# Sin3DM/Sin3DM

Hardware: AMD Instinct MI355X
Metric: DDPM-1000 triplane samples/sec @128^2 latent (higher is better)
Workload: dtype f32; 1 GPU; BASELINE configs[1]: 128^2 triplane (H,W,D)=(128,128,128), 128-ch TriplaneUNetModelSmall, DDPM-1000, batch 1 per GPU; a step = 1 denoising step; batch_per_gpu=1, parallelism=1 independent samples, prewarm_steps=150

## Files before the change

### include/sin3dm_hip.h

```cpp
#ifndef SIN3DM_HIP_H
#define SIN3DM_HIP_H

#include <stddef.h>
#include <stdint.h>

#ifdef __cplusplus
extern "C" {
#endif

#define S3D_ABI_VERSION 13
#define S3D_API __attribute__((visibility("default")))

typedef enum {
    S3D_OK = 0,
    S3D_ERR_INVALID = -1,
    S3D_ERR_MISSING = -2,
    S3D_ERR_HIP = -3,
    S3D_ERR_UNSUPPORTED = -4,
    S3D_ERR_INTERNAL = -5
} s3d_status;

S3D_API int s3d_abi_version(void);

S3D_API int s3d_set_option(const char* name, const char* value);
S3D_API int s3d_get_option(const char* name, int* value);
S3D_API int s3d_set_riders(int on);
S3D_API const char* s3d_last_error(void);
S3D_API int s3d_device_count(void);

typedef struct s3d_unet s3d_unet;

typedef struct {
    int32_t in_channels;
    int32_t model_channels;
    int32_t out_channels;
    int32_t num_res_blocks;
    int32_t n_levels;
    int32_t channel_mult[8];
    int32_t use_scale_shift_norm;
    int32_t is_rollout;
} s3d_unet_cfg;
// ... 18 lines not shown
S3D_API int s3d_unet_forward_film(s3d_unet* m, const float* x, const float* film, int film_stride, int B, int H, int W, int D,
                          float* out, void* stream);

#define S3D_PROF_CLASSES 4
typedef struct {
    double ms[S3D_PROF_CLASSES];
    double flops[S3D_PROF_CLASSES];
    int64_t launches[S3D_PROF_CLASSES];
    int64_t forwards;
    double mfma_flops[S3D_PROF_CLASSES];
} s3d_profile;
S3D_API int s3d_unet_profile(s3d_unet* m, int every);
S3D_API int s3d_unet_profile_classes(s3d_unet* m, int mask);
S3D_API int s3d_unet_profile_read(s3d_unet* m, s3d_profile* out);
S3D_API const char* s3d_unet_profile_kernel(const s3d_unet* m, int cls);
enum { S3D_TAB_SQRT_RECIP = 0, S3D_TAB_SQRT_RECIPM1, S3D_TAB_COEF1, S3D_TAB_COEF2, S3D_TAB_LOGVAR,
       S3D_TAB_ACP, S3D_TAB_ACP_PREV, S3D_TAB_ROWS };
enum { S3D_STEP_DDPM = 0, S3D_STEP_DDIM = 1, S3D_STEP_MEAN_ONLY = 2 };
enum { S3D_MEAN_START_X = 0, S3D_MEAN_EPSILON = 1 };

typedef struct {
    int32_t mode;
    int32_t mean_type;
    int32_t clip_denoised;
    int32_t is_mask_t0;
    float eta;
    int32_t T;
    int64_t batch;
    int64_t per_sample;
    const float* model_out;
// ... 237 lines not shown
```

### sin3dm_amd/_lib.py

```python
from __future__ import annotations

import ctypes as C
import os

_HERE = os.path.dirname(os.path.abspath(__file__))
LIB_PATH = os.path.join(_HERE, "libsin3dm_hip.so")

c_fp = C.POINTER(C.c_float)
c_i64p = C.POINTER(C.c_int64)

ABI_VERSION = 13
TAB_ROWS = ("sqrt_recip", "sqrt_recipm1", "coef1", "coef2", "logvar", "acp", "acp_prev")
KTAB_ROWS = ("sqrt_acp_prev", "sqrt_1m_acp_prev", "sqrt_1m_beta", "sqrt_beta")
STEP_DDPM, STEP_DDIM, STEP_MEAN_ONLY = 0, 1, 2
CARRY_OUT, CARRY_IN = 1, 2
MEAN_START_X, MEAN_EPSILON = 0, 1
ERR_INVALID, ERR_MISSING, ERR_HIP, ERR_UNSUPPORTED, ERR_INTERNAL = -1, -2, -3, -4, -5
MAX_LANES = 16
MESHSDF_MAX_PAIRS = 1 << 27
RENDER_MAX_PAIRS = 1 << 27
RENDER_TILE, RENDER_SUBPIXEL, RENDER_MAX_COORD, RENDER_MAX_GRID = 16, 256, 1 << 20, 4096
IMGFEAT_INCEPTION, IMGFEAT_ALEXNET = 0, 1
RENDER_AMBIENT, RENDER_DIFFUSE = 0.35, 0.65

# ... 29 lines not shown
                ("tex_threshold_ratio", C.c_float), ("tex_weight", C.c_float)]


class DecoderCfg(C.Structure):
    _fields_ = [("geo_feat_channels", C.c_int32), ("tex_feat_channels", C.c_int32), ("feat_channel_up", C.c_int32),
                ("mlp_hidden_channels", C.c_int32), ("mlp_hidden_layers", C.c_int32), ("tex_channels", C.c_int32)]


SIGNATURES = {
    "s3d_abi_version": (C.c_int, []),
    "s3d_last_error": (C.c_char_p, []),
    "s3d_device_count": (C.c_int, []),
    "s3d_set_option": (C.c_int, [C.c_char_p, C.c_char_p]),
    "s3d_get_option": (C.c_int, [C.c_char_p, C.POINTER(C.c_int)]),
    "s3d_set_riders": (C.c_int, [C.c_int]),
    "s3d_unet_create": (C.c_int, [C.POINTER(UNetCfg), C.POINTER(C.c_void_p)]),
    "s3d_unet_destroy": (None, [C.c_void_p]),
    "s3d_unet_num_params": (C.c_int, [C.c_void_p]),
    "s3d_unet_param_info": (C.c_int, [C.c_void_p, C.c_int, C.POINTER(C.c_char_p), c_i64p, C.POINTER(C.c_int)]),
    "s3d_unet_set_param": (C.c_int, [C.c_void_p, C.c_char_p, C.c_void_p, c_i64p, C.c_int]),
    "s3d_unet_forward": (C.c_int, [C.c_void_p, C.c_void_p, C.c_void_p, C.c_int, C.c_int, C.c_int, C.c_int,
                                   C.c_void_p, C.c_void_p]),
    "s3d_unet_film_width": (C.c_int, [C.c_void_p]),
    "s3d_unet_film": (C.c_int, [C.c_void_p, C.c_void_p, C.c_int, C.c_void_p, C.c_void_p]),
    "s3d_unet_select_lane": (C.c_int, [C.c_void_p, C.c_int]),
    "s3d_unet_current_lane": (C.c_int, [C.c_void_p]),
    "s3d_unet_forward_film": (C.c_int, [C.c_void_p, C.c_void_p, C.c_void_p, C.c_int, C.c_int, C.c_int, C.c_int, C.c_int,
                                        C.c_void_p, C.c_void_p]),
    "s3d_unet_profile": (C.c_int, [C.c_void_p, C.c_int]),
    "s3d_unet_profile_classes": (C.c_int, [C.c_void_p, C.c_int]),
    "s3d_unet_profile_read": (C.c_int, [C.c_void_p, C.POINTER(Profile)]),
    "s3d_unet_profile_kernel": (C.c_char_p, [C.c_void_p, C.c_int]),
    "s3d_sampler_step": (C.c_int, [C.POINTER(SamplerArgs), C.c_void_p]),
    "s3d_unet_step_film": (C.c_int, [C.c_void_p, C.c_void_p, C.c_int, C.c_int, C.c_int, C.c_int, C.c_int,
                                     C.POINTER(SamplerArgs), C.c_void_p, C.c_void_p]),
    "s3d_unet_step_film_carry": (C.c_int, [C.c_void_p, C.c_void_p, C.c_int, C.c_int, C.c_int, C.c_int, C.c_int,
                                           C.POINTER(SamplerArgs), C.c_void_p, C.c_void_p, C.c_int]),
    "s3d_sampler_step_known": (C.c_int, [C.POINTER(SamplerArgs), C.POINTER(KnownRegionArgs), C.c_void_p]),
    "s3d_unet_step_film_known": (C.c_int, [C.c_void_p, C.c_void_p, C.c_int, C.c_int, C.c_int, C.c_int, C.c_int,
                                           C.POINTER(SamplerArgs), C.POINTER(KnownRegionArgs), C.c_void_p, C.c_void_p, C.c_int]),
    "s3d_sampler_renoise": (C.c_int, [C.c_void_p, C.c_void_p, C.c_void_p, C.c_void_p, C.c_int32, C.c_int64, C.c_int64, C.c_void_p,
                                      C.c_void_p]),
    "s3d_op_triplane_conv": (C.c_int, [C.POINTER(C.c_void_p), C.POINTER(C.c_void_p), C.c_int, C.c_int, C.c_int,
                                       C.c_int, C.c_int, C.c_int, C.c_int, C.c_int, C.POINTER(C.c_void_p),
                                       C.POINTER(C.c_void_p), C.c_void_p]),
    "s3d_op_triplane_norm_silu": (C.c_int, [C.POINTER(C.c_void_p), C.POINTER(C.c_void_p), C.c_int, C.c_int, C.c_int,
                                            C.c_int, C.c_int, C.POINTER(C.c_void_p), C.POINTER(C.c_void_p),
# ... 180 lines not shown
    if not torch.cuda.is_available():
        raise Sin3DMHipError("sin3dm_amd needs a visible MI355X (torch.cuda.is_available() is False); "
                             "there is no CPU fallback")


def set_option(name, value):
    check(load().s3d_set_option(str(name).encode(), None if value is None else str(value).encode()))


def get_option(name):
    v = C.c_int(0)
    check(load().s3d_get_option(str(name).encode(), C.byref(v)))
    return None if v.value == -1 else v.value


def set_riders(on):
    check(load().s3d_set_riders(1 if on else 0))


def stream_ptr():
    import torch
    return C.c_void_p(torch.cuda.current_stream().cuda_stream)


def ptr(t):
    return C.c_void_p(t.data_ptr()) if t is not None else C.c_void_p(0)


def ptr3(ts):
    return (C.c_void_p * 3)(*[C.c_void_p(t.data_ptr()) for t in ts])
# ... 1 lines not shown
```

### sin3dm_amd/csrc/s3d_common.h

```cpp
#pragma once
#include <hip/hip_runtime.h>

#include <atomic>
#include <cstdarg>
#include <cstdint>
#include <cstdio>
#include <cstring>
#include <map>
#include <string>
#include <vector>

#include "../../include/sin3dm_hip.h"

namespace s3d {

void set_error(const char* fmt, ...) __attribute__((format(printf, 1, 2)));
const char* get_error();

#define S3D_HIP(call)                                                                              \
    do {                                                                                           \
        hipError_t e__ = (call);                                                                   \
        if (e__ != hipSuccess) {                                                                   \
            s3d::set_error("%s failed: %s (%s:%d)", #call, hipGetErrorString(e__), __FILE__, __LINE__); \
            return S3D_ERR_HIP;                                                                    \
// ... 138 lines not shown
    const float* u[3];
    int hi[3], wi[3];
    int C, cq, pl, sg, nsub, maxparts;
    double* part;
};
struct GnFinCatArgs {
    const double* pu; const double* ps; float* mr;
    int maxparts_u, maxparts_s, nparts_u[3], nparts_s[3], nsub_u, nsub_s, subs_per_group;
    double count[3];
};
enum RiderKind { RIDER_NONE = 0, RIDER_GN_PARTIALS_UP, RIDER_GN_FINALIZE, RIDER_GN_FINALIZE_CAT };
struct ConvRider {
    int kind;
    int n_blocks;
    int gx;
    union { GnPartUpArgs up; GnFinArgs fin; GnFinCatArgs cat; };
};
constexpr int kRiderLdsBytes = 16384;
int launch_conv(ConvKind kind, ConvArgs& a, hipStream_t st, const ConvRider* rider = nullptr);
bool conv1x1_takes_rider(const Geo& g, int B, int cout);
int launch_conv_naive(ConvKind kind, ConvArgs& a, hipStream_t st);
bool conv_use_naive();
void conv_note_kernel(const char* name);
const char* conv_last_kernel();
double conv_exec_fraction(ConvKind kind, const ConvArgs& a);

struct ConvW {
    size_t dense[3] = {0, 0, 0};
    size_t bias[3] = {0, 0, 0};
    size_t rrow[3] = {0, 0, 0};
// ... 48 lines not shown
bool conv_use_wino24();
bool conv_wino24_channels(int cin, int cout);
size_t wino24_packed_floats(int cout, int cin);
size_t pack_wino24s_weights(std::vector<float>& stage, const float* W, int cout, int ctot, int cin);
int launch_conv_wino24s(ConvArgs& a, hipStream_t st);
int launch_conv_wino24_narrow(ConvArgs& a, hipStream_t st);
int launch_conv_wino24_wide(ConvArgs& a, hipStream_t st);

struct ActArgs {
    const float* gamma[3];
    const float* beta[3];
    const float* film;
    int film_stride;
};
constexpr int kActRows = 8, kActCols = 8;
struct MeanPartials {
    float* rowpart[3];
    float* colpart[3];
};
int launch_gn_act(const Tri& x, int B, GnStats stats, const ActArgs& a, Tri& y, const MeanPartials* mp,
                  hipStream_t st, const GnPartials* stats_part = nullptr);
bool gn_act_can_add_parts(const GnPartials& part, int C);
bool gn_parts_in_consumer(long long consumer_blocks);
int gn_act_threads(int C);
long long gn_act_blocks(const Geo& g, int B);
int launch_gn_finalize_as(const GnPartials& part, const Geo& g, int C, int B, int threads, GnStats out, hipStream_t st);
int launch_gn_act_cat(const Tri& u, const Tri& sk, int B, GnStats stats, const ActArgs& a, Tri& y, const MeanPartials* mp,
                      hipStream_t st);
struct MeanVecs { float* rowmean[3]; float* colmean[3]; };
struct MeanFinArgs {
// ... 40 lines not shown
```

### sin3dm_amd/csrc/s3d_conv.hip

```cpp
#include "s3d_common.h"
#include "s3d_rank1.h"
#include "s3d_riders.h"

namespace s3d {

typedef float f32x16 __attribute__((ext_vector_type(16)));

#ifndef S3D_ABLATE
#define S3D_ABLATE 0
#endif
constexpr int KC = 32;
constexpr int LDP = KC + 4;

__device__ __forceinline__ float up2x_blend(float ly0, float ly1, float lx0, float lx1, float v00, float v01, float v10, float v11) {
    const float top = __fmaf_rn(lx1, v01, __fmul_rn(lx0, v00));
    const float bot = __fmaf_rn(lx1, v11, __fmul_rn(lx0, v10));
    return __fmaf_rn(ly1, bot, __fmul_rn(ly0, top));
}

template <int TH_, int TW_, int KH_, int KW_, int WM_, int WN_, int MTW_, int NTW_, int KS_ = 1, int PF_ = 0, bool TR_ = false>
struct ConvCfg {
    static constexpr int KS = KS_;
    static constexpr int PF = PF_;
    static constexpr bool TR = TR_;
// ... 18 lines not shown

template <bool RIDER> struct RiderArg {};
template <> struct RiderArg<true> { ConvRider r; };
template <class CFG, bool RIDER = false>
__global__ __launch_bounds__(256) void k_conv_mfma(ConvArgs args, RiderArg<RIDER> rider) {
    constexpr int TW = CFG::TW, KH = CFG::KH, KW = CFG::KW, MTW = CFG::MTW, NTW = CFG::NTW;
    constexpr int HW = CFG::HW, TAPS = KH * KW;
    __shared__ __attribute__((aligned(16))) float smem[2 * (CFG::A_ELEMS + CFG::B_ELEMS)];
    float* const Abase = smem;
    float* const Bbase = smem + 2 * CFG::A_ELEMS;

    int bid = blockIdx.x;
    int nblocks = gridDim.x;
    if constexpr (RIDER) {
        static_assert(sizeof smem >= size_t(kRiderLdsBytes) && KH == 1 && !CFG::TR, "the rider bodies work in the 1x1 convolution's LDS");
        if (bid < rider.r.n_blocks) { run_rider(rider.r, bid, smem); return; }
        bid -= rider.r.n_blocks; nblocks -= rider.r.n_blocks;
    }
    if (args.xcd_swizzle) {
        const int chunk = nblocks >> 3;
        if (bid < (chunk << 3)) bid = (bid & 7) * chunk + (bid >> 3);
    }
    int j = 0;
#pragma unroll
    for (int k = 1; k < kMaxConvJobs; ++k) j += (k < args.njobs && bid >= args.job[k].block_begin) ? 1 : 0;
    const ConvJob& J = args.job[j];
    int local = bid - J.block_begin;
    const int ntile = local % J.n_tiles_n; local /= J.n_tiles_n;
    const int b = local / J.tiles_per_img; local %= J.tiles_per_img;
    const int ty0 = (local / J.tiles_x) * CFG::TH, tx0 = (local % J.tiles_x) * TW;
    const int n0 = ntile * CFG::BN;
    const int h = J.h, w = J.w, cin = args.cin, cout = args.cout;
// ... 724 lines not shown
```

### sin3dm_amd/csrc/s3d_kernels.hip

```cpp
#include "s3d_common.h"
#include "s3d_rank1.h"
#include "s3d_riders.h"
#include "s3d_sampler.h"

namespace s3d {

__device__ __forceinline__ float silu_f(float v) { return v * __builtin_amdgcn_rcpf(1.0f + __expf(-v)); }

static inline int cdiv(int a, int b) { return (a + b - 1) / b; }

__global__ void k_nchw_to_nhwc(const float* __restrict__ in, float* __restrict__ out, int B, int C, int hw) {
    size_t i = size_t(blockIdx.x) * blockDim.x + threadIdx.x;
    size_t n = size_t(B) * C * hw;
    if (i >= n) return;
    int c = int(i % C);
    size_t r = i / C;
    int pix = int(r % hw);
    int b = int(r / hw);
    out[i] = in[(size_t(b) * C + c) * hw + pix];
}
__global__ void k_nhwc_to_nchw(const float* __restrict__ in, float* __restrict__ out, int B, int C, int hw) {
    size_t i = size_t(blockIdx.x) * blockDim.x + threadIdx.x;
    size_t n = size_t(B) * C * hw;
    if (i >= n) return;
// ... 213 lines not shown

__global__ __launch_bounds__(256) void k_gn_finalize(GnFinArgs a) {
    __shared__ double sm4[4];
    gn_finalize_block(a, blockIdx.x, blockIdx.y, blockIdx.z, sm4);
}
static bool gn_finalize_args(const GnPartials& part, const Geo& g, int C, GnStats out, GnFinArgs& a) {
    a.part = part.p; a.mr = out.mr; a.maxparts = part.maxparts; a.nsub = part.nsub;
    if (part.nsub % 32 != 0) return false;
    a.subs_per_group = part.nsub / 32;
    for (int p = 0; p < 3; ++p) { a.nparts[p] = part.nparts[p]; a.count[p] = double(C / 32) * g.h[p] * g.w[p]; }
    return true;
}
bool gn_finalize_rider(const GnPartials& part, const Geo& g, int C, int B, GnStats out, ConvRider& r) {
    memset(&r, 0, sizeof r);
    if (!B || !gn_finalize_args(part, g, C, out, r.fin)) return false;
    r.kind = RIDER_GN_FINALIZE; r.gx = 32; r.n_blocks = 32 * 3 * B;
    return true;
}
int launch_gn_finalize(const GnPartials& part, const Geo& g, int C, int B, GnStats out, hipStream_t st) {
    GnFinArgs a;
    S3D_CHECK(gn_finalize_args(part, g, C, out, a), S3D_ERR_INVALID, "gn_finalize: nsub=%d", part.nsub);
    if (!B) return 0;
    hipLaunchKernelGGL(k_gn_finalize, dim3(32, 3, B), dim3(256), 0, st, a);
    S3D_HIP(hipGetLastError());
    return 0;
}

__device__ __forceinline__ float4 up2x_sample(const float4* __restrict__ src, int hi, int wi, int cuq, int yo, int xo) {
    float fy = 0.5f * (float(yo) + 0.5f) - 0.5f; fy = fy < 0.f ? 0.f : fy;
    float fx = 0.5f * (float(xo) + 0.5f) - 0.5f; fx = fx < 0.f ? 0.f : fx;
    int y0 = int(fy); y0 = y0 > hi - 1 ? hi - 1 : y0;
// ... 30 lines not shown
int launch_gn_partials_up(const Tri& u, int B, int sg, GnPartials out, hipStream_t st) {
    GnPartUpArgs a;
    int maxtiles = 0;
    S3D_CHECK(gn_partials_up_args(u, sg, out, a, maxtiles), S3D_ERR_INVALID, "gn_partials_up: layout");
    if (!maxtiles || !B) return 0;
    hipLaunchKernelGGL(k_gn_partials_up, dim3(maxtiles, 3, B), dim3(a.cq * a.pl), size_t(a.pl) * a.C * 2 * sizeof(double), st, a);
    S3D_HIP(hipGetLastError());
    return 0;
}
bool gn_partials_up_rider(const Tri& u, int B, int sg, GnPartials out, ConvRider& r) {
    memset(&r, 0, sizeof r);
    int maxtiles = 0;
    if (!gn_partials_up_args(u, sg, out, r.up, maxtiles) || !maxtiles || !B) return false;
    if (r.up.cq * r.up.pl != 256 || size_t(r.up.pl) * r.up.C * 2 * sizeof(double) > size_t(kRiderLdsBytes)) return false;
    r.kind = RIDER_GN_PARTIALS_UP; r.gx = maxtiles; r.n_blocks = maxtiles * 3 * B;
    return true;
}
__global__ __launch_bounds__(256) void k_gn_finalize_cat(GnFinCatArgs a) {
    __shared__ double sm4[4];
    gn_finalize_cat_block(a, blockIdx.x, blockIdx.y, blockIdx.z, sm4);
}
static bool gn_finalize_cat_args(const GnPartials& pu, const GnPartials& ps, const Geo& g, int C, GnStats out, GnFinCatArgs& a) {
    a.pu = pu.p; a.ps = ps.p; a.mr = out.mr; a.maxparts_u = pu.maxparts; a.maxparts_s = ps.maxparts; a.nsub_u = pu.nsub; a.nsub_s = ps.nsub;
    if ((pu.nsub + ps.nsub) % 32 != 0) return false;
    a.subs_per_group = (pu.nsub + ps.nsub) / 32;
    for (int p = 0; p < 3; ++p) { a.nparts_u[p] = pu.nparts[p]; a.nparts_s[p] = ps.nparts[p]; a.count[p] = double(C / 32) * g.h[p] * g.w[p]; }
    return true;
}
bool gn_finalize_cat_rider(const GnPartials& pu, const GnPartials& ps, const Geo& g, int C, int B, GnStats out, ConvRider& r) {
    memset(&r, 0, sizeof r);
    if (!B || !gn_finalize_cat_args(pu, ps, g, C, out, r.cat)) return false;
    r.kind = RIDER_GN_FINALIZE_CAT; r.gx = 32; r.n_blocks = 32 * 3 * B;
    return true;
}
int launch_gn_finalize_cat(const GnPartials& pu, const GnPartials& ps, const Geo& g, int C, int B, GnStats out, hipStream_t st) {
    GnFinCatArgs a;
    S3D_CHECK(gn_finalize_cat_args(pu, ps, g, C, out, a), S3D_ERR_INVALID, "gn_finalize_cat: nsub=%d+%d", pu.nsub, ps.nsub);
    if (!B) return 0;
    hipLaunchKernelGGL(k_gn_finalize_cat, dim3(32, 3, B), dim3(256), 0, st, a);
    S3D_HIP(hipGetLastError());
    return 0;
}

struct GnPartSrc { const double* part; int nparts[3], maxparts, nsub, spg; double count[3]; };
__device__ __forceinline__ float* gn_stats_from_parts(const GnPartSrc& a, int b, int p, double* sd, float* mr_out) {
    const int L = int(blockDim.x) >> 5, tid = threadIdx.x;
    if (tid < 32 * L) {
// ... 51 lines not shown
    hipLaunchKernelGGL(k_gn_finalize_as, dim3(3, B), dim3(threads), size_t(threads) * 2 * sizeof(double) + 64 * sizeof(float), st, ps, out.mr);
    S3D_HIP(hipGetLastError());
    return 0;
}

struct GnActArgs {
    const float* x[3]; float* y[3];
    const float* gamma[3]; const float* beta[3];
    float* rowpart[3]; float* colpart[3];
    const float* mr;
    const float* film; int film_stride;
    int h[3], w[3];
    int C, cq, pl, with_means;
    GnPartSrc ps;
    float* mr_out;
};
__global__ __launch_bounds__(256) void k_gn_act(GnActArgs a) {
    extern __shared__ __attribute__((aligned(16))) char smem_raw[];
    float* sm = reinterpret_cast<float*>(smem_raw);
    const int p = blockIdx.y, b = blockIdx.z;
    const int h = a.h[p], w = a.w[p];
    const int ntc = (w + kActCols - 1) / kActCols, ntr = (h + kActRows - 1) / kActRows;
    if (int(blockIdx.x) >= ntc * ntr) return;
    const int tr = blockIdx.x / ntc, tc = blockIdx.x % ntc;
    const bool ident = a.mr == nullptr && a.ps.part == nullptr;
    const int q = threadIdx.x % a.cq, l = threadIdx.x / a.cq;
    const int i0 = tr * kActRows, j0 = tc * kActCols;
    const int i1 = min(h, i0 + kActRows), j1 = min(w, j0 + kActCols);
    const float4* xs = reinterpret_cast<const float4*>(a.x[p] + size_t(b) * h * w * a.C) + q;
    float4* ys = reinterpret_cast<float4*>(a.y[p] + size_t(b) * h * w * a.C) + q;
    float4 xfirst[kActRows];
    {
        const int j = min(j0 + l, j1 - 1);
#pragma unroll
        for (int r = 0; r < kActRows; ++r) xfirst[r] = xs[(size_t(min(i0 + r, i1 - 1)) * w + j) * a.cq];
    }
    const bool film = a.film != nullptr;
    float4 gam4 = make_float4(1, 1, 1, 1), bet4 = make_float4(0, 0, 0, 0), fsc4 = make_float4(0, 0, 0, 0), fsh4 = make_float4(0, 0, 0, 0);
    if (!ident) { gam4 = reinterpret_cast<const float4*>(a.gamma[p])[q]; bet4 = reinterpret_cast<const float4*>(a.beta[p])[q]; }
    if (film) {
        fsc4 = reinterpret_cast<const float4*>(a.film + size_t(b) * a.film_stride)[q];
// ... 15 lines not shown
        const float s1[4] = {fsc4.x, fsc4.y, fsc4.z, fsc4.w}, s2[4] = {fsh4.x, fsh4.y, fsh4.z, fsh4.w};
#pragma unroll
        for (int k = 0; k < 4; ++k) {
            const int c = 4 * q + k, g = c / cg;
            const float scale = ident ? 1.0f : sm[32 + g] * gv[k];
            A[k] = scale;
            Bc[k] = ident ? 0.0f : bv[k] - scale * sm[g];
            sc[k] = film ? 1.0f + s1[k] : 1.0f;
            sh[k] = film ? s2[k] : 0.0f;
        }
    }
    __syncthreads();
    float4 rowacc[kActRows];
#pragma unroll
    for (int r = 0; r < kActRows; ++r) rowacc[r] = make_float4(0, 0, 0, 0);
    for (int j = j0 + l; j < j1; j += a.pl) {
        float4 colacc = make_float4(0, 0, 0, 0);
        float4 xin[kActRows];
        if (j == j0 + l) {
#pragma unroll
            for (int r = 0; r < kActRows; ++r) xin[r] = xfirst[r];
        } else {
#pragma unroll
            for (int r = 0; r < kActRows; ++r) xin[r] = xs[(size_t(min(i0 + r, i1 - 1)) * w + j) * a.cq];
        }
#pragma unroll
        for (int r = 0; r < kActRows; ++r) {
            const int i = i0 + r;
            if (i < i1) {
                const size_t off = (size_t(i) * w + j) * a.cq;
                const float4 v = xin[r];
                float4 o;
                o.x = fmaf(v.x, A[0], Bc[0]); o.y = fmaf(v.y, A[1], Bc[1]);
                o.z = fmaf(v.z, A[2], Bc[2]); o.w = fmaf(v.w, A[3], Bc[3]);
// ... 1 lines not shown
                    o.x = o.x * sc[0] + sh[0]; o.y = o.y * sc[1] + sh[1];
                    o.z = o.z * sc[2] + sh[2]; o.w = o.w * sc[3] + sh[3];
                }
                if (!ident) { o.x = silu_f(o.x); o.y = silu_f(o.y); o.z = silu_f(o.z); o.w = silu_f(o.w); }
                ys[off] = o;
                colacc.x += o.x; colacc.y += o.y; colacc.z += o.z; colacc.w += o.w;
                rowacc[r].x += o.x; rowacc[r].y += o.y; rowacc[r].z += o.z; rowacc[r].w += o.w;
            }
        }
        if (a.with_means)
            reinterpret_cast<float4*>(a.colpart[p] + ((size_t(b) * ntr + tr) * w + j) * a.C)[q] = colacc;
    }
    if (!a.with_means) return;
    float4* smr = reinterpret_cast<float4*>(smem_raw);
#pragma unroll
    for (int r = 0; r < kActRows; ++r) smr[(size_t(l) * kActRows + r) * a.cq + q] = rowacc[r];
    __syncthreads();
    const int nthr = a.cq * a.pl;
    for (int it = threadIdx.x; it < kActRows * a.cq; it += nthr) {
        const int r = it / a.cq, qq = it % a.cq;
        const int i = i0 + r;
        if (i >= i1) continue;
        float4 s = make_float4(0, 0, 0, 0);
        for (int ll = 0; ll < a.pl; ++ll) {
            const float4 v = smr[(size_t(ll) * kActRows + r) * a.cq + qq];
            s.x += v.x; s.y += v.y; s.z += v.z; s.w += v.w;
        }
        reinterpret_cast<float4*>(a.rowpart[p] + ((size_t(b) * ntc + tc) * h + i) * a.C)[qq] = s;
    }
}
bool gn_act_can_add_parts(const GnPartials& part, int C) {
    if (!part.p || part.nsub % 32 != 0 || C % 32 != 0) return false;
    return (part.nsub / 32) * part.maxparts <= 160;
}
bool gn_parts_in_consumer(long long consumer_blocks) {
    const int mode = opt(OPT_GN_FUSED);
    const int cus = device_cus();
    return mode < 0 ? consumer_blocks <= 6LL * cus : mode != 0;
}
int gn_act_threads(int C) { int cq, pl; thread_shape(C, cq, pl); return cq * std::min(pl, kActCols); }
long long gn_act_blocks(const Geo& g, int B) {
    int maxtiles = 0;
    for (int p = 0; p < 3; ++p) maxtiles = std::max(maxtiles, cdiv(g.h[p], kActRows) * cdiv(g.w[p], kActCols));
// ... 9 lines not shown
        a.ps = gn_part_src(*stats_part, x.g, x.C);
    }
    int maxtiles = 0;
    for (int p = 0; p < 3; ++p) {
        a.x[p] = x.p[p]; a.y[p] = y.p[p]; a.h[p] = x.g.h[p]; a.w[p] = x.g.w[p];
        a.gamma[p] = aa.gamma[p]; a.beta[p] = aa.beta[p];
        a.rowpart[p] = mp ? mp->rowpart[p] : nullptr;
        a.colpart[p] = mp ? mp->colpart[p] : nullptr;
        maxtiles = std::max(maxtiles, cdiv(a.h[p], kActRows) * cdiv(a.w[p], kActCols));
    }
    a.mr = stats.mr; a.film = aa.film; a.film_stride = aa.film_stride;
    a.C = x.C; thread_shape(x.C, a.cq, a.pl); a.with_means = mp ? 1 : 0;
    a.pl = std::min(a.pl, kActCols);
    S3D_CHECK(x.C % 32 == 0 && a.cq * a.pl <= 256, S3D_ERR_INVALID, "GroupNorm(32, C): C=%d unsupported", x.C);
    if (!maxtiles || !B) return 0;
    size_t shm = std::max(size_t(64) * sizeof(float), size_t(a.pl) * kActRows * a.C * sizeof(float));
    if (a.ps.part) shm = std::max(shm, size_t(a.cq) * a.pl * 2 * sizeof(double) + 64 * sizeof(float));
    hipLaunchKernelGGL(k_gn_act, dim3(maxtiles, 3, B), dim3(a.cq * a.pl), shm, st, a);
    S3D_HIP(hipGetLastError());
    return 0;
}

struct GnActCatArgs {
    GnActArgs base;
    const float* u[3]; const float* sk[3];
    int cuq, csq;
};
__global__ __launch_bounds__(512) void k_gn_act_cat(GnActCatArgs ca) {
    const GnActArgs& a = ca.base;
    extern __shared__ __attribute__((aligned(16))) char smem_raw[];
    float* sm = reinterpret_cast<float*>(smem_raw);
    const int p = blockIdx.y, b = blockIdx.z;
    const int h = a.h[p], w = a.w[p];
// ... 98 lines not shown
    int maxtiles = 0;
    for (int p = 0; p < 3; ++p) {
        a.x[p] = nullptr; a.y[p] = y.p[p]; a.h[p] = y.g.h[p]; a.w[p] = y.g.w[p];
        ca.u[p] = u.p[p]; ca.sk[p] = sk.p[p];
        a.gamma[p] = aa.gamma[p]; a.beta[p] = aa.beta[p];
        a.rowpart[p] = mp ? mp->rowpart[p] : nullptr;
        a.colpart[p] = mp ? mp->colpart[p] : nullptr;
        maxtiles = std::max(maxtiles, cdiv(a.h[p], kActRows) * cdiv(a.w[p], kActCols));
        S3D_CHECK(y.g.h[p] == 2 * u.g.h[p] && y.g.w[p] == 2 * u.g.w[p] && sk.g.h[p] == y.g.h[p] && sk.g.w[p] == y.g.w[p], S3D_ERR_INVALID, "gn_act_cat: geometry");
    }
    ca.cuq = u.C / 4; ca.csq = sk.C / 4;
    a.mr = stats.mr; a.film = aa.film; a.film_stride = aa.film_stride;
    a.C = y.C; thread_shape(y.C, a.cq, a.pl); a.with_means = mp ? 1 : 0;
    S3D_CHECK(y.C == u.C + sk.C && y.C % 32 == 0 && a.cq * a.pl <= 512 && stats.mr, S3D_ERR_INVALID, "gn_act_cat: C=%d unsupported", y.C);
    if (!maxtiles || !B) return 0;
    size_t shm = std::max(size_t(64) * sizeof(float), size_t(a.pl) * kActRows * a.C * sizeof(float));
    hipLaunchKernelGGL(k_gn_act_cat, dim3(maxtiles, 3, B), dim3(a.cq * a.pl), shm, st, ca);
    S3D_HIP(hipGetLastError());
    return 0;
}

__global__ __launch_bounds__(256) void k_means_finalize(MeanFinArgs a) {
    means_finalize_thread(a, blockIdx.y, blockIdx.z, int(blockIdx.x * 128 + threadIdx.x));
}
MeanFinArgs means_finalize_args(const Geo& g, int C, int B, const MeanPartials& mp, const MeanVecs& mv) {
    MeanFinArgs a;
    a.C = C; a.cq = C / 4; a.B = B;
    for (int p = 0; p < 3; ++p) {
        const int h = g.h[p], w = g.w[p];
        a.src[2 * p] = mp.rowpart[p]; a.dst[2 * p] = mv.rowmean[p];
// ... 746 lines not shown
```

### sin3dm_amd/csrc/s3d_model.h

```cpp
#pragma once
#include <algorithm>
#include <cmath>
#include <memory>

#include "s3d_common.h"

namespace s3d {

static const char* kPlane[3] = {"xy", "xz", "yz"};

struct ParamSpec {
    std::string name;
    std::vector<int64_t> shape;
    size_t numel() const { size_t n = 1; for (auto d : shape) n *= size_t(d); return n; }
};

struct NormW { size_t gamma[3], beta[3]; };
struct ResBlockW {
    std::string prefix;
    int C, Cout;
    NormW n1, n2;
    ConvW c1, c2, skip;
    ConvW skip_a, skip_b;
    int c_up = 0;
// ... 100 lines not shown
    struct ProfRec { int cls; hipEvent_t e0, e1; double flops, mfma_flops; };
    int prof_every = 0;
    long fwd_count = 0;
    bool prof_now = false;
    int prof_mask = 15;
    bool prof_train = false;
    std::vector<ProfRec> prof_recs;
    std::vector<hipEvent_t> prof_pool;
    int64_t prof_forwards = 0;
    std::string prof_kernel[S3D_PROF_CLASSES];
    void note_prof_kernel(int cls) {
        if (cls < 0 || cls >= S3D_PROF_CLASSES) return;
        const std::string n = conv_last_kernel();
        if (n.empty() || prof_kernel[cls].find(n) != std::string::npos) return;
        prof_kernel[cls] += (prof_kernel[cls].empty() ? "" : " + ") + n;
    }
    hipEvent_t prof_event() {
        hipEvent_t e = nullptr;
        if (!prof_pool.empty()) { e = prof_pool.back(); prof_pool.pop_back(); }
        else if (hipEventCreate(&e) != hipSuccess) e = nullptr;
        return e;
    }
    int timed_conv(int cls, ConvKind kind, ConvArgs& ca, hipStream_t st, const ConvRider* rider = nullptr) {
        if (!prof_now || !((prof_mask >> cls) & 1)) return launch_conv(kind, ca, st, rider);
        int taps = kind == CONV_3x3 ? 9 : (kind == CONV_1x1 ? 1 : (kind == CONV_1x3_VEC ? 3 : (kind == CONV_1x3_ROLL ? 9 : 25)));
        double pix = 0;
        for (int j = 0; j < ca.njobs; ++j) pix += double(ca.job[j].h) * ca.job[j].w;
        ProfRec r{cls, prof_event(), prof_event(), 2.0 * taps * ca.cin * ca.cout * pix * ca.B, 0.0};
        r.mfma_flops = r.flops * conv_exec_fraction(kind, ca);
        if (r.e0) (void)hipEventRecord(r.e0, st);
// ... 133 lines not shown
            if (!measuring) S3D_TRY(launch_gn_finalize_as(x.part, x.g, x.C, B, gn_act_threads(x.C), stats, st));
        } else if (!add_parts) S3D_TRY(stats_of(x, stats));
        else if (nt) stats.mr = ar().alloc<float>(size_t(B) * 3 * 64);
        if (nt) { nt->stats = stats; nt->roll = cw && cw->rollout; }
        y = alloc_tri(x.C, x.g);
        ActArgs aa;
        for (int p = 0; p < 3; ++p) { aa.gamma[p] = m->dev(nw.gamma[p]); aa.beta[p] = m->dev(nw.beta[p]); }
        aa.film = film_ptr; aa.film_stride = fstride();
        const bool roll = cw && cw->rollout;
        MeanPartials mp; MeanVecs mv;
        if (roll) S3D_TRY(roll_buffers(y, *cw, true, mp, mv, rrow, rcol));
        else for (int p = 0; p < 3; ++p) { rrow[p] = rcol[p] = nullptr; }
        if (nt && roll) nt->mv = mv;
        if (measuring) return 0;
        S3D_TRY(launch_gn_act(x, B, stats, aa, y, roll ? &mp : nullptr, st, add_parts ? &x.part : nullptr));
        if (!roll) return 0;
        return rank1_tables(y, *cw, mp, mv, rrow, rcol);
    }

    bool riders_on() const { return !tape && riders_enabled() && opt_on(OPT_VCAT); }
    bool rides(const ConvW& cw, const Geo& g) const { return riders_on() && cw.k == 1 && conv1x1_takes_rider(g, B, cw.cout); }

    int conv(const Tri& y, const ConvW& cw, const float* bbias, const float* const rrow[3], const float* const rcol[3],
             const Tri* res, Tri& out, int want_stats = 0, hipStream_t on = nullptr, bool no_bias = false, bool res_up = false,
             const ConvRider* rider = nullptr) {
        hipStream_t st = on ? on : this->st;
        out = alloc_tri(cw.cout, y.g);
        if (!(cw.k == 3 && !conv_use_naive())) want_stats = 0;
        const bool w24 = cw.k == 3 && cw.wino24s[0] != 0 && conv_wino24_channels(cw.cin, cw.cout);
        S3D_CHECK(!(cw.only24_current && (!w24 || conv_use_naive())), S3D_ERR_INVALID,
// ... 49 lines not shown
            if (!up_rides) S3D_TRY(launch_gn_partials_up(u, B, sg, pu, st));
            if (!fin_rides) S3D_TRY(launch_gn_finalize_cat(pu, sk.part, sk.g, C, B, stats, st));
        }
        Tri y1, h1, y2;
        y1 = alloc_tri(C, sk.g);
        const float *rr[3], *rc[3];
        {
            ActArgs aa;
            for (int p = 0; p < 3; ++p) { aa.gamma[p] = m->dev(rb.n1.gamma[p]); aa.beta[p] = m->dev(rb.n1.beta[p]); }
            aa.film = nullptr; aa.film_stride = fstride();
            const bool roll = rb.c1.rollout;
            MeanPartials mp; MeanVecs mv;
            S3D_TRY(roll_buffers(y1, rb.c1, roll, mp, mv, rr, rc));
            if (!measuring) {
                S3D_TRY(launch_gn_act_cat(u, sk, B, stats, aa, y1, roll ? &mp : nullptr, st));
                if (roll) S3D_TRY(rank1_tables(y1, rb.c1, mp, mv, rr, rc));
            }
        }
        S3D_TRY(conv(y1, rb.c1, ssn ? nullptr : film_ptr, rr, rc, nullptr, h1, 2));
        S3D_TRY(norm_act(h1, rb.n2, ssn ? film_ptr : nullptr, &rb.c2, y2, rr, rc, nullptr));
        S3D_TRY(conv(y2, rb.c2, nullptr, rr, rc, &skip, out, out_stats));
        return 0;
    }

    int resblock(const ResBlockW& rb, const Tri& x, Tri& out, bool out_feeds_norm, int out_stats_override = -1, const ChunkStats* fin = nullptr) {
        const bool ssn = m->cfg.use_scale_shift_norm != 0;
        const float* film_ptr = film ? film + rb.film_off : nullptr;
        Tri y1, h1, y2;
        const float *rr[3], *rc[3];
        Tri skip;
// ... 24 lines not shown
```

### sin3dm_amd/csrc/s3d_runtime.hip

```cpp
#include "s3d_common.h"
#include <atomic>

namespace s3d {

static thread_local char g_err[1024] = "";

void set_error(const char* fmt, ...) {
    va_list ap;
    va_start(ap, fmt);
    vsnprintf(g_err, sizeof g_err, fmt, ap);
    va_end(ap);
}
const char* get_error() { return g_err; }

int DevBuf::reserve(size_t bytes) {
    if (bytes <= cap) return 0;
    release();
    S3D_HIP(hipMalloc(&p, bytes));
    cap = bytes;
    return 0;
}
void DevBuf::release() {
    if (p) (void)hipFree(p);
    p = nullptr;
// ... 41 lines not shown
    if (strncmp(name, "S3D_", 4) == 0) name += 4;
    for (int o = 0; o < OPT_COUNT; ++o) if (strcmp(name, kOptNames[o]) == 0) return o;
    return -1;
}
static std::atomic<int> g_riders{-1};
bool riders_enabled() {
    int v = g_riders.load(std::memory_order_acquire);
    if (v < 0) {
        const char* e = getenv("S3D_RIDERS");
        int expect = -1;
        g_riders.compare_exchange_strong(expect, e && strcmp(e, "0") == 0 ? 0 : 1, std::memory_order_acq_rel);
        v = g_riders.load(std::memory_order_acquire);
    }
    return v != 0;
}
int device_cus() {
    static std::atomic<int> cache[64];
    int dev = 0;
    if (hipGetDevice(&dev) != hipSuccess || dev < 0 || dev >= 64) dev = 0;
    int n = cache[dev].load(std::memory_order_relaxed);
    if (n > 0) return n;
    n = 256;
    if (hipDeviceGetAttribute(&n, hipDeviceAttributeMultiprocessorCount, dev) != hipSuccess || n <= 0) n = 256;
    cache[dev].store(n, std::memory_order_relaxed);
    return n;
}

}

extern "C" {
// ... 9 lines not shown
    g_opt_state[o].store(2, std::memory_order_release);
    g_opt_gen.fetch_add(1, std::memory_order_acq_rel);
    return 0;
}

int s3d_get_option(const char* name, int* value) {
    using namespace s3d;
    const int o = find_opt(name);
    S3D_CHECK(o >= 0 && value, S3D_ERR_INVALID, "get_option: unknown option '%s'", name ? name : "(null)");
    *value = opt(Opt(o));
    return 0;
}

int s3d_set_riders(int on) {
    s3d::g_riders.store(on ? 1 : 0, std::memory_order_release);
    return 0;
}

int s3d_abi_version(void) { return S3D_ABI_VERSION; }
const char* s3d_last_error(void) { return s3d::get_error(); }

int s3d_device_count(void) {
    int n = 0;
    hipError_t e = hipGetDeviceCount(&n);
    if (e != hipSuccess) {
        s3d::set_error("hipGetDeviceCount failed: %s", hipGetErrorString(e));
        return S3D_ERR_HIP;
    }
    return n;
}
// ... 40 lines not shown
```

### sin3dm_amd/csrc/s3d_unet.hip

```cpp
#include "s3d_model.h"


namespace s3d {

static void add_lin(std::vector<ParamSpec>& s, const std::string& p, int o, int i) {
    s.push_back({p + ".weight", {o, i}});
    s.push_back({p + ".bias", {o}});
}
static void add_tconv(std::vector<ParamSpec>& s, const std::string& p, int cin, int cout, int k, bool roll) {
    for (int i = 0; i < 3; ++i) {
        s.push_back({p + ".conv_" + kPlane[i] + ".weight", {cout, roll ? 3 * cin : cin, k, k}});
        s.push_back({p + ".conv_" + kPlane[i] + ".bias", {cout}});
    }
}
static void add_tnorm(std::vector<ParamSpec>& s, const std::string& p, int c) {
    for (int i = 0; i < 3; ++i) {
        s.push_back({p + ".norm_" + kPlane[i] + ".weight", {c}});
        s.push_back({p + ".norm_" + kPlane[i] + ".bias", {c}});
    }
}
static void add_resblock(std::vector<ParamSpec>& s, const std::string& p, int c, int cout, int ted, bool ssn, bool roll) {
    add_tnorm(s, p + ".in_layers.0", c);
    add_tconv(s, p + ".in_layers.2", c, cout, 3, roll);
    add_lin(s, p + ".emb_layers.1", ssn ? 2 * cout : cout, ted);
// ... 501 lines not shown
    ++m->fwd_count;
    if (m->prof_now) ++m->prof_forwards;
    m->arena.peak = 0;
    rc = run_forward(m, x, t, B, H, W, D, out, st, nullptr, ext_film, ext_film_stride, fuse, carry_flags, known);
    m->prof_now = false;
    if (rc) return rc;
    return workspace_overrun("unet_forward", m->arena.peak, m->inf_high);
}

extern "C" {

int s3d_unet_profile(s3d_unet* m, int every) {
    S3D_CHECK(m && every >= 0, S3D_ERR_INVALID, "unet_profile: bad argument");
    m->prof_every = every;
    m->fwd_count = 0;
    if (every > 0)
        for (int c = 0; c < S3D_PROF_CLASSES; ++c) if ((m->prof_mask >> c) & 1) m->prof_kernel[c].clear();
    return 0;
}

int s3d_unet_profile_classes(s3d_unet* m, int mask) {
    S3D_CHECK(m && mask >= 0 && mask < (1 << S3D_PROF_CLASSES), S3D_ERR_INVALID, "unet_profile_classes: bad argument");
    m->prof_mask = mask;
    return 0;
}

int s3d_unet_profile_read(s3d_unet* m, s3d_profile* out) {
    S3D_CHECK(m && out, S3D_ERR_INVALID, "unet_profile_read: null argument");
    for (auto& r : m->prof_recs) {
        if (r.e0 && r.e1) {
            S3D_HIP(hipEventSynchronize(r.e1));
            float ms = 0.f;
// ... 4 lines not shown
            out->launches[r.cls] += 1;
        }
        if (r.e0) m->prof_pool.push_back(r.e0);
        if (r.e1) m->prof_pool.push_back(r.e1);
    }
    m->prof_recs.clear();
    out->forwards += m->prof_forwards;
    m->prof_forwards = 0;
    return 0;
}

const char* s3d_unet_profile_kernel(const s3d_unet* m, int cls) {
    return m && cls >= 0 && cls < S3D_PROF_CLASSES ? m->prof_kernel[cls].c_str() : "";
}

}
```

### sin3dm_amd/diffusion/unet_triplane.py

```python
from __future__ import annotations

import ctypes as C
import os

import torch as th
import torch.nn as nn

from .. import _lib
from ..testing import unet_param_shapes


class _Node(nn.Module):
    """Anonymous container used to rebuild the reference's dotted parameter names."""


def _register(root, dotted, tensor):
    parts = dotted.split(".")
    mod = root
    for p in parts[:-1]:
        if p not in mod._modules:
            mod.add_module(p, _Node())
        mod = mod._modules[p]
    mod.register_parameter(parts[-1], nn.Parameter(tensor))

# ... 217 lines not shown
                pass

    def profile(self, every, classes=7):
        lib = self._ensure_handle()
        _lib.check(lib.s3d_unet_profile_classes(self._handle, int(classes)))
        _lib.check(lib.s3d_unet_profile(self._handle, int(every)))

    def profile_read(self, into=None):
        prof = into if into is not None else _lib.Profile()
        _lib.check(_lib.load().s3d_unet_profile_read(self._handle, C.byref(prof)))
        return prof

    def profile_kernel(self, cls=0):
        return (_lib.load().s3d_unet_profile_kernel(self._handle, int(cls)) or b"").decode()

    def convert_to_fp16(self):
        raise NotImplementedError("fp16 is not runnable in the reference (see __init__)")

    def convert_to_fp32(self):
        pass

    def forward(self, x, timesteps, H=None, W=None, D=None, y=None):
        assert H is not None and W is not None and D is not None
        _lib.require_gpu(x)
        if y is not None:
            x = th.cat([x, y], dim=1)
        if th.is_grad_enabled() and any(p.requires_grad for p in self.parameters()):
            self._ensure_flat()
            names = [n for n, _, _, _ in self._flat_layout]
            params = dict(self.named_parameters())
# ... 137 lines not shown
```

Measured before the change: 1.199 samples/s.

## Split GroupNorm-activation kernel into 128-channel slices on small grids

Adds a templated split variant of k_gn_act in which each block handles one 128-channel slice of a spatial tile. It is used when the unsplit grid has at most three blocks per CU, so low-occupancy levels launch more blocks to fill the GPU. Row-mean partials are reduced per slice. Partials-up rider blocks are also moved to the end of the conv grid instead of the front. This adds an env or API toggle and profiling hooks that record which act kernel ran. The cost is more blocks, each reloading the tile's edges.

```diff
diff --git a/include/sin3dm_hip.h b/include/sin3dm_hip.h
--- a/include/sin3dm_hip.h
+++ b/include/sin3dm_hip.h
@@ -25,6 +25,7 @@
 S3D_API int s3d_set_option(const char* name, const char* value);
 S3D_API int s3d_get_option(const char* name, int* value);
 S3D_API int s3d_set_riders(int on);
+S3D_API int s3d_set_act_split(int on);
 S3D_API const char* s3d_last_error(void);
 S3D_API int s3d_device_count(void);
 
@@ -73,6 +74,7 @@
 S3D_API int s3d_unet_profile_classes(s3d_unet* m, int mask);
 S3D_API int s3d_unet_profile_read(s3d_unet* m, s3d_profile* out);
 S3D_API const char* s3d_unet_profile_kernel(const s3d_unet* m, int cls);
+S3D_API const char* s3d_unet_act_kernels(const s3d_unet* m);
 enum { S3D_TAB_SQRT_RECIP = 0, S3D_TAB_SQRT_RECIPM1, S3D_TAB_COEF1, S3D_TAB_COEF2, S3D_TAB_LOGVAR,
        S3D_TAB_ACP, S3D_TAB_ACP_PREV, S3D_TAB_ROWS };
 enum { S3D_STEP_DDPM = 0, S3D_STEP_DDIM = 1, S3D_STEP_MEAN_ONLY = 2 };
diff --git a/sin3dm_amd/_lib.py b/sin3dm_amd/_lib.py
--- a/sin3dm_amd/_lib.py
+++ b/sin3dm_amd/_lib.py
@@ -67,6 +67,7 @@
     "s3d_set_option": (C.c_int, [C.c_char_p, C.c_char_p]),
     "s3d_get_option": (C.c_int, [C.c_char_p, C.POINTER(C.c_int)]),
     "s3d_set_riders": (C.c_int, [C.c_int]),
+    "s3d_set_act_split": (C.c_int, [C.c_int]),
     "s3d_unet_create": (C.c_int, [C.POINTER(UNetCfg), C.POINTER(C.c_void_p)]),
     "s3d_unet_destroy": (None, [C.c_void_p]),
     "s3d_unet_num_params": (C.c_int, [C.c_void_p]),
@@ -84,6 +85,7 @@
     "s3d_unet_profile_classes": (C.c_int, [C.c_void_p, C.c_int]),
     "s3d_unet_profile_read": (C.c_int, [C.c_void_p, C.POINTER(Profile)]),
     "s3d_unet_profile_kernel": (C.c_char_p, [C.c_void_p, C.c_int]),
+    "s3d_unet_act_kernels": (C.c_char_p, [C.c_void_p]),
     "s3d_sampler_step": (C.c_int, [C.POINTER(SamplerArgs), C.c_void_p]),
     "s3d_unet_step_film": (C.c_int, [C.c_void_p, C.c_void_p, C.c_int, C.c_int, C.c_int, C.c_int, C.c_int,
                                      C.POINTER(SamplerArgs), C.c_void_p, C.c_void_p]),
@@ -294,6 +296,10 @@
     return None if v.value == -1 else v.value
 
 
+def set_act_split(on):
+    check(load().s3d_set_act_split(1 if on else 0))
+
+
 def set_riders(on):
     check(load().s3d_set_riders(1 if on else 0))
 
diff --git a/sin3dm_amd/csrc/s3d_common.h b/sin3dm_amd/csrc/s3d_common.h
--- a/sin3dm_amd/csrc/s3d_common.h
+++ b/sin3dm_amd/csrc/s3d_common.h
@@ -176,6 +176,7 @@
     int kind;
     int n_blocks;
     int gx;
+    int last;
     union { GnPartUpArgs up; GnFinArgs fin; GnFinCatArgs cat; };
 };
 constexpr int kRiderLdsBytes = 16384;
@@ -254,6 +255,9 @@
     int film_stride;
 };
 constexpr int kActRows = 8, kActCols = 8;
+constexpr int kActSliceQuads = 32;
+bool act_split_enabled();
+bool act_split_for(long long unsplit_blocks);
 struct MeanPartials {
     float* rowpart[3];
     float* colpart[3];
diff --git a/sin3dm_amd/csrc/s3d_conv.hip b/sin3dm_amd/csrc/s3d_conv.hip
--- a/sin3dm_amd/csrc/s3d_conv.hip
+++ b/sin3dm_amd/csrc/s3d_conv.hip
@@ -56,8 +56,10 @@
     int nblocks = gridDim.x;
     if constexpr (RIDER) {
         static_assert(sizeof smem >= size_t(kRiderLdsBytes) && KH == 1 && !CFG::TR, "the rider bodies work in the 1x1 convolution's LDS");
-        if (bid < rider.r.n_blocks) { run_rider(rider.r, bid, smem); return; }
-        bid -= rider.r.n_blocks; nblocks -= rider.r.n_blocks;
+        const int nr = rider.r.n_blocks, first = rider.r.last ? nblocks - nr : 0;
+        if (bid >= first && bid < first + nr) { run_rider(rider.r, bid - first, smem); return; }
+        if (!rider.r.last) bid -= nr;
+        nblocks -= nr;
     }
     if (args.xcd_swizzle) {
         const int chunk = nblocks >> 3;
diff --git a/sin3dm_amd/csrc/s3d_kernels.hip b/sin3dm_amd/csrc/s3d_kernels.hip
--- a/sin3dm_amd/csrc/s3d_kernels.hip
+++ b/sin3dm_amd/csrc/s3d_kernels.hip
@@ -251,7 +251,7 @@
 bool gn_finalize_rider(const GnPartials& part, const Geo& g, int C, int B, GnStats out, ConvRider& r) {
     memset(&r, 0, sizeof r);
     if (!B || !gn_finalize_args(part, g, C, out, r.fin)) return false;
-    r.kind = RIDER_GN_FINALIZE; r.gx = 32; r.n_blocks = 32 * 3 * B;
+    r.kind = RIDER_GN_FINALIZE; r.gx = 32; r.n_blocks = 32 * 3 * B; r.last = 0;
     return true;
 }
 int launch_gn_finalize(const GnPartials& part, const Geo& g, int C, int B, GnStats out, hipStream_t st) {
@@ -312,6 +312,7 @@
     if (!gn_partials_up_args(u, sg, out, r.up, maxtiles) || !maxtiles || !B) return false;
     if (r.up.cq * r.up.pl != 256 || size_t(r.up.pl) * r.up.C * 2 * sizeof(double) > size_t(kRiderLdsBytes)) return false;
     r.kind = RIDER_GN_PARTIALS_UP; r.gx = maxtiles; r.n_blocks = maxtiles * 3 * B;
+    r.last = 1;
     return true;
 }
 __global__ __launch_bounds__(256) void k_gn_finalize_cat(GnFinCatArgs a) {
@@ -328,7 +329,7 @@
 bool gn_finalize_cat_rider(const GnPartials& pu, const GnPartials& ps, const Geo& g, int C, int B, GnStats out, ConvRider& r) {
     memset(&r, 0, sizeof r);
     if (!B || !gn_finalize_cat_args(pu, ps, g, C, out, r.cat)) return false;
-    r.kind = RIDER_GN_FINALIZE_CAT; r.gx = 32; r.n_blocks = 32 * 3 * B;
+    r.kind = RIDER_GN_FINALIZE_CAT; r.gx = 32; r.n_blocks = 32 * 3 * B; r.last = 0;
     return true;
 }
 int launch_gn_finalize_cat(const GnPartials& pu, const GnPartials& ps, const Geo& g, int C, int B, GnStats out, hipStream_t st) {
@@ -410,17 +411,34 @@
     int C, cq, pl, with_means;
     GnPartSrc ps;
     float* mr_out;
+    int nslice;
 };
+__device__ __forceinline__ float4 act_row_meet_split(const float4* smr, int r, int qq, int pl) {
+    float4 s = make_float4(0, 0, 0, 0);
+    for (int ll = 0; ll < pl; ++ll) {
+        float4 t = make_float4(0, 0, 0, 0);
+        for (int k = ll; k < kActCols; k += pl) {
+            const float4 v = smr[(size_t(k) * kActRows + r) * kActSliceQuads + qq];
+            t.x += v.x; t.y += v.y; t.z += v.z; t.w += v.w;
+        }
+        s.x += t.x; s.y += t.y; s.z += t.z; s.w += t.w;
+    }
+    return s;
+}
+template <bool SPLIT>
 __global__ __launch_bounds__(256) void k_gn_act(GnActArgs a) {
     extern __shared__ __attribute__((aligned(16))) char smem_raw[];
     float* sm = reinterpret_cast<float*>(smem_raw);
     const int p = blockIdx.y, b = blockIdx.z;
     const int h = a.h[p], w = a.w[p];
     const int ntc = (w + kActCols - 1) / kActCols, ntr = (h + kActRows - 1) / kActRows;
-    if (int(blockIdx.x) >= ntc * ntr) return;
-    const int tr = blockIdx.x / ntc, tc = blockIdx.x % ntc;
+    const int tile = SPLIT ? int(blockIdx.x) / a.nslice : int(blockIdx.x);
+    const int slice = SPLIT ? int(blockIdx.x) - tile * a.nslice : 0;
+    if (tile >= ntc * ntr) return;
+    const int tr = tile / ntc, tc = tile % ntc;
     const bool ident = a.mr == nullptr && a.ps.part == nullptr;
-    const int q = threadIdx.x % a.cq, l = threadIdx.x / a.cq;
+    const int cqb = SPLIT ? kActSliceQuads : a.cq, plb = SPLIT ? kActCols : a.pl;
+    const int ql = threadIdx.x % cqb, l = threadIdx.x / cqb, q = slice * kActSliceQuads + ql;
     const int i0 = tr * kActRows, j0 = tc * kActCols;
     const int i1 = min(h, i0 + kActRows), j1 = min(w, j0 + kActCols);
     const float4* xs = reinterpret_cast<const float4*>(a.x[p] + size_t(b) * h * w * a.C) + q;
@@ -466,10 +484,10 @@
     float4 rowacc[kActRows];
 #pragma unroll
     for (int r = 0; r < kActRows; ++r) rowacc[r] = make_float4(0, 0, 0, 0);
-    for (int j = j0 + l; j < j1; j += a.pl) {
+    for (int j = j0 + l; j < j1; j += plb) {
         float4 colacc = make_float4(0, 0, 0, 0);
         float4 xin[kActRows];
-        if (j == j0 + l) {
+        if (SPLIT || j == j0 + l) {
 #pragma unroll
             for (int r = 0; r < kActRows; ++r) xin[r] = xfirst[r];
         } else {
@@ -501,19 +519,20 @@
     if (!a.with_means) return;
     float4* smr = reinterpret_cast<float4*>(smem_raw);
 #pragma unroll
-    for (int r = 0; r < kActRows; ++r) smr[(size_t(l) * kActRows + r) * a.cq + q] = rowacc[r];
+    for (int r = 0; r < kActRows; ++r) smr[(size_t(l) * kActRows + r) * cqb + ql] = rowacc[r];
     __syncthreads();
-    const int nthr = a.cq * a.pl;
-    for (int it = threadIdx.x; it < kActRows * a.cq; it += nthr) {
-        const int r = it / a.cq, qq = it % a.cq;
+    const int nthr = cqb * plb;
+    for (int it = threadIdx.x; it < kActRows * cqb; it += nthr) {
+        const int r = it / cqb, qq = it % cqb;
         const int i = i0 + r;
         if (i >= i1) continue;
         float4 s = make_float4(0, 0, 0, 0);
-        for (int ll = 0; ll < a.pl; ++ll) {
+        if (SPLIT) s = act_row_meet_split(smr, r, qq, a.pl);
+        else for (int ll = 0; ll < a.pl; ++ll) {
             const float4 v = smr[(size_t(ll) * kActRows + r) * a.cq + qq];
             s.x += v.x; s.y += v.y; s.z += v.z; s.w += v.w;
         }
-        reinterpret_cast<float4*>(a.rowpart[p] + ((size_t(b) * ntc + tc) * h + i) * a.C)[qq] = s;
+        reinterpret_cast<float4*>(a.rowpart[p] + ((size_t(b) * ntc + tc) * h + i) * a.C)[slice * kActSliceQuads + qq] = s;
     }
 }
 bool gn_act_can_add_parts(const GnPartials& part, int C) {
@@ -553,9 +572,20 @@
     a.pl = std::min(a.pl, kActCols);
     S3D_CHECK(x.C % 32 == 0 && a.cq * a.pl <= 256, S3D_ERR_INVALID, "GroupNorm(32, C): C=%d unsupported", x.C);
     if (!maxtiles || !B) return 0;
+    a.nslice = act_split_for((long long)maxtiles * 3 * B) && x.C > kActSliceQuads * 4 && x.C % (kActSliceQuads * 4) == 0 && a.cq * a.pl == 256
+                   ? x.C / (kActSliceQuads * 4) : 1;
+    if (a.nslice > 1) {
+        conv_note_kernel("k_gn_act<split> (128-channel slices)");
+        size_t shm = size_t(kActCols) * kActRows * kActSliceQuads * sizeof(float4);
+        if (a.ps.part) shm = std::max(shm, size_t(256) * 2 * sizeof(double) + 64 * sizeof(float));
+        hipLaunchKernelGGL(k_gn_act<true>, dim3(maxtiles * a.nslice, 3, B), dim3(256), shm, st, a);
+        S3D_HIP(hipGetLastError());
+        return 0;
+    }
+    conv_note_kernel("k_gn_act (all channels)");
     size_t shm = std::max(size_t(64) * sizeof(float), size_t(a.pl) * kActRows * a.C * sizeof(float));
     if (a.ps.part) shm = std::max(shm, size_t(a.cq) * a.pl * 2 * sizeof(double) + 64 * sizeof(float));
-    hipLaunchKernelGGL(k_gn_act, dim3(maxtiles, 3, B), dim3(a.cq * a.pl), shm, st, a);
+    hipLaunchKernelGGL(k_gn_act<false>, dim3(maxtiles, 3, B), dim3(a.cq * a.pl), shm, st, a);
     S3D_HIP(hipGetLastError());
     return 0;
 }
@@ -684,6 +714,7 @@
     a.C = y.C; thread_shape(y.C, a.cq, a.pl); a.with_means = mp ? 1 : 0;
     S3D_CHECK(y.C == u.C + sk.C && y.C % 32 == 0 && a.cq * a.pl <= 512 && stats.mr, S3D_ERR_INVALID, "gn_act_cat: C=%d unsupported", y.C);
     if (!maxtiles || !B) return 0;
+    conv_note_kernel("k_gn_act_cat");
     size_t shm = std::max(size_t(64) * sizeof(float), size_t(a.pl) * kActRows * a.C * sizeof(float));
     hipLaunchKernelGGL(k_gn_act_cat, dim3(maxtiles, 3, B), dim3(a.cq * a.pl), shm, st, ca);
     S3D_HIP(hipGetLastError());
diff --git a/sin3dm_amd/csrc/s3d_model.h b/sin3dm_amd/csrc/s3d_model.h
--- a/sin3dm_amd/csrc/s3d_model.h
+++ b/sin3dm_amd/csrc/s3d_model.h
@@ -138,6 +138,13 @@
         const std::string n = conv_last_kernel();
         if (n.empty() || prof_kernel[cls].find(n) != std::string::npos) return;
         prof_kernel[cls] += (prof_kernel[cls].empty() ? "" : " + ") + n;
+    }
+    std::string prof_act;
+    void note_act_kernel() {
+        if (!prof_now) return;
+        const std::string n = conv_last_kernel();
+        if (n.empty() || prof_act.find(n) != std::string::npos) return;
+        prof_act += (prof_act.empty() ? "" : " + ") + n;
     }
     hipEvent_t prof_event() {
         hipEvent_t e = nullptr;
@@ -301,6 +308,7 @@
         if (nt && roll) nt->mv = mv;
         if (measuring) return 0;
         S3D_TRY(launch_gn_act(x, B, stats, aa, y, roll ? &mp : nullptr, st, add_parts ? &x.part : nullptr));
+        m->note_act_kernel();
         if (!roll) return 0;
         return rank1_tables(y, *cw, mp, mv, rrow, rcol);
     }
@@ -380,6 +388,7 @@
             S3D_TRY(roll_buffers(y1, rb.c1, roll, mp, mv, rr, rc));
             if (!measuring) {
                 S3D_TRY(launch_gn_act_cat(u, sk, B, stats, aa, y1, roll ? &mp : nullptr, st));
+                m->note_act_kernel();
                 if (roll) S3D_TRY(rank1_tables(y1, rb.c1, mp, mv, rr, rc));
             }
         }
diff --git a/sin3dm_amd/csrc/s3d_runtime.hip b/sin3dm_amd/csrc/s3d_runtime.hip
--- a/sin3dm_amd/csrc/s3d_runtime.hip
+++ b/sin3dm_amd/csrc/s3d_runtime.hip
@@ -79,6 +79,18 @@
     }
     return v != 0;
 }
+static std::atomic<int> g_act_split{-1};
+bool act_split_enabled() {
+    int v = g_act_split.load(std::memory_order_acquire);
+    if (v < 0) {
+        const char* e = getenv("S3D_ACT_SPLIT");
+        int expect = -1;
+        g_act_split.compare_exchange_strong(expect, e && strcmp(e, "0") == 0 ? 0 : 1, std::memory_order_acq_rel);
+        v = g_act_split.load(std::memory_order_acquire);
+    }
+    return v != 0;
+}
+bool act_split_for(long long unsplit_blocks) { return act_split_enabled() && unsplit_blocks <= 3LL * device_cus(); }
 int device_cus() {
     static std::atomic<int> cache[64];
     int dev = 0;
@@ -118,6 +130,11 @@
 
 int s3d_set_riders(int on) {
     s3d::g_riders.store(on ? 1 : 0, std::memory_order_release);
+    return 0;
+}
+
+int s3d_set_act_split(int on) {
+    s3d::g_act_split.store(on ? 1 : 0, std::memory_order_release);
     return 0;
 }
 
diff --git a/sin3dm_amd/csrc/s3d_unet.hip b/sin3dm_amd/csrc/s3d_unet.hip
--- a/sin3dm_amd/csrc/s3d_unet.hip
+++ b/sin3dm_amd/csrc/s3d_unet.hip
@@ -539,8 +539,10 @@
     S3D_CHECK(m && every >= 0, S3D_ERR_INVALID, "unet_profile: bad argument");
     m->prof_every = every;
     m->fwd_count = 0;
-    if (every > 0)
+    if (every > 0) {
         for (int c = 0; c < S3D_PROF_CLASSES; ++c) if ((m->prof_mask >> c) & 1) m->prof_kernel[c].clear();
+        m->prof_act.clear();
+    }
     return 0;
 }
 
@@ -575,4 +577,6 @@
     return m && cls >= 0 && cls < S3D_PROF_CLASSES ? m->prof_kernel[cls].c_str() : "";
 }
 
-}
+const char* s3d_unet_act_kernels(const s3d_unet* m) { return m ? m->prof_act.c_str() : ""; }
+
+}
diff --git a/sin3dm_amd/diffusion/unet_triplane.py b/sin3dm_amd/diffusion/unet_triplane.py
--- a/sin3dm_amd/diffusion/unet_triplane.py
+++ b/sin3dm_amd/diffusion/unet_triplane.py
@@ -255,6 +255,9 @@
     def profile_kernel(self, cls=0):
         return (_lib.load().s3d_unet_profile_kernel(self._handle, int(cls)) or b"").decode()
 
+    def act_kernels(self):
+        return (_lib.load().s3d_unet_act_kernels(self._handle) or b"").decode()
+
     def convert_to_fp16(self):
         raise NotImplementedError("fp16 is not runnable in the reference (see __init__)")
 
```

After: 1.201 samples/s (median of 6 runs). About the same (+0.2%).
